# mfalxa/fakepta

Hardware: AMD Instinct MI355X
Metric: residual samples/sec (TOA×realization) for 100-psr HD GWB; % FP64 peak (higher is better)
Workload: dtype f64

## Files before the change

### fakepta_amd/csrc/fused_sched.h

```cpp
#pragma once
#include <cstdint>

#if defined(__HIPCC__)
#define FPTA_SCHED_HD __host__ __device__
#else
#define FPTA_SCHED_HD
#endif

namespace fpta {

constexpr int kFusedShapeAny = 0;
constexpr int kFusedShapeGenLoad = 1;
constexpr int kFusedShapeLoad = 2;
constexpr int kFusedSlotAny = -1, kFusedSlotNone = 0, kFusedSlotGen = 1, kFusedSlotLoad = 2;
FPTA_SCHED_HD constexpr int fused_shape_nsig(int shape) {
  return shape == kFusedShapeGenLoad ? 2 : shape == kFusedShapeLoad ? 1 : 0;
}
FPTA_SCHED_HD constexpr int fused_shape_slot(int shape, int s, int i) {
  return shape == kFusedShapeAny       ? kFusedSlotAny
         : shape == kFusedShapeGenLoad ? (i == 0 ? kFusedSlotGen : (s == 0 && i == 1 ? kFusedSlotLoad : kFusedSlotNone))
                                       : (s == 0 && i == 0 ? kFusedSlotLoad : kFusedSlotNone);
}

FPTA_SCHED_HD constexpr int fused_shape_match(int n_sig, const int32_t* n_terms, const int32_t (*kind)[2]) {
  return n_sig == 2 && n_terms[0] == 2 && kind[0][0] == 0 && kind[0][1] == 1 && n_terms[1] == 1 && kind[1][0] == 0
             ? kFusedShapeGenLoad
         : n_sig == 1 && n_terms[0] == 1 && kind[0][0] == 1 ? kFusedShapeLoad
                                                            : kFusedShapeAny;
}

FPTA_SCHED_HD constexpr int32_t fused_ksteps(int32_t nm, int par) { return (((nm + (par ? 0 : 1)) >> 1) + 3) >> 2; }
FPTA_SCHED_HD constexpr int32_t fused_groups(int32_t nm) { return (fused_ksteps(nm, 0) + 1) >> 1; }

FPTA_SCHED_HD constexpr int32_t fused_iterations(int32_t ng0, int32_t ng1) { return ng0 > ng1 ? ng0 : ng1; }
FPTA_SCHED_HD constexpr bool fused_steps(int32_t jng, int32_t g) { return g < jng; }
FPTA_SCHED_HD constexpr bool fused_draw_loads(int32_t ng_s, int32_t g, bool last) { return last || g + 1 < ng_s; }
FPTA_SCHED_HD constexpr bool fused_draws(int32_t ng_s, int32_t g, bool last, bool nx) { return last ? nx : g + 1 < ng_s; }
FPTA_SCHED_HD constexpr int32_t fused_draw_group(int32_t g, bool last) { return last ? 0 : g + 1; }

}

#undef FPTA_SCHED_HD
```

### fakepta_amd/csrc/grid_fused.hip

```cpp
#include <hip/hip_runtime.h>
#include <hip/hip_ext.h>
#include <algorithm>
#include <atomic>
#include <type_traits>

#include "fused_device.h"

namespace fpta {

#ifndef FPTA_FUSED_DFT_PRIO
#define FPTA_FUSED_DFT_PRIO 3
#endif
#ifndef FPTA_HALF_STORE16
#define FPTA_HALF_STORE16 0
#endif
#ifndef FPTA_HALF_AHEAD
#define FPTA_HALF_AHEAD 2
#endif
constexpr int kFusedHalfAhead = FPTA_HALF_AHEAD;
#ifndef FPTA_HALF_PIN
#define FPTA_HALF_PIN 0
#endif

#ifndef FPTA_FUSED_CUT
#define FPTA_FUSED_CUT 0
#endif

namespace {

template <int NS>
struct FusedOps {
  int c;
  i32x4 ci;
  dbl2 b[NS];
  int row[NS];
};
template <int NS>
struct FusedOpsH {
  int c;
  i32x4 ci;
  dbl2 b[2][NS / 2];
  int row[2][NS];
};

__device__ __forceinline__ uint32_t dpp_u32_xor1(uint32_t x) {
  return (uint32_t)__builtin_amdgcn_update_dpp(0, (int)x, 0xB1, 0xF, 0xF, false);
}
__device__ __forceinline__ void bm_half(uint32_t wl, uint32_t wa, double& zc, double& zs) {
  double sn, cs;
  const double r = bm_sqrt(-2.0 * bm_log_u32(wl));
  bm_sincos2pi_u32(wa, sn, cs);
  zc = r * cs;
  zs = r * sn;
}
__device__ __forceinline__ void fused_mix_tile(const FusedMix& m, int k, int rg, int pg, int lane) {
  constexpr int NT = kFusedMixGroup / 16;
  const int lr = lane & 15, lg = lane >> 4;
  const int r = 16 * rg + lr;
  const bool rv = r < m.n_real;
  const uint64_t g = (uint64_t)(m.real0 + r);
  const int p0 = kFusedMixGroup * pg;
  int qe[NT];
  int qmax = 0;
#pragma unroll
  for (int t = 0; t < NT; ++t) {
    const int pt = p0 + 16 * t;
    qe[t] = pt < m.P ? min(m.lower ? min(m.P, pt + 16) : m.P, m.n_q) : 0;
    qmax = max(qmax, qe[t]);
  }
  d4 acc[NT][2];
#pragma unroll
  for (int t = 0; t < NT; ++t) acc[t][0] = acc[t][1] = d4{0.0, 0.0, 0.0, 0.0};
  const double* __restrict__ lt = m.LT + p0 + lr;
  const bool paired = (m.real0 & 1) == 0;
  const int e = lr & 1;
  const uint32_t ctr3 = (uint32_t)(g >> 1);
  for (int q0 = 0; q0 < qmax; q0 += 8) {
    double a0[NT], a1[NT];
#pragma unroll
    for (int t = 0; t < NT; ++t) {
      a0[t] = q0 < qe[t] ? ld_global(lt + (int64_t)(q0 + lg) * m.lt_ld + 16 * t) : 0.0;
      a1[t] = q0 + 4 < qe[t] ? ld_global(lt + (int64_t)(q0 + 4 + lg) * m.lt_ld + 16 * t) : 0.0;
    }
    double zc0, zs0, zc1, zs1;
    if (paired) {
      const u32x4 v = philox4x32_10({(uint32_t)k, (uint32_t)(q0 + 4 * e + lg), (uint32_t)m.seg, ctr3}, m.k0, m.k1);
      const uint32_t r0 = dpp_u32_xor1(e ? v.x : v.z), r1 = dpp_u32_xor1(e ? v.y : v.w);
      bm_half(e ? r0 : v.x, e ? r1 : v.y, zc0, zs0);
      bm_half(e ? v.z : r0, e ? v.w : r1, zc1, zs1);
    } else {
      gp_normal2((uint32_t)k, (uint32_t)(q0 + lg), (uint32_t)m.seg, g, m.k0, m.k1, zc0, zs0);
      gp_normal2((uint32_t)k, (uint32_t)(q0 + 4 + lg), (uint32_t)m.seg, g, m.k0, m.k1, zc1, zs1);
    }
    const bool ok0 = rv && q0 + lg < m.n_q, ok1 = rv && q0 + 4 + lg < m.n_q;
    zc0 = ok0 ? zc0 : 0.0;
    zs0 = ok0 ? zs0 : 0.0;
    zc1 = ok1 ? zc1 : 0.0;
    zs1 = ok1 ? zs1 : 0.0;
#pragma unroll
    for (int t = 0; t < NT; ++t)
      if (q0 < qe[t]) {
        acc[t][0] = __builtin_amdgcn_mfma_f64_16x16x4f64(a0[t], zc0, acc[t][0], 0, 0, 0);
        acc[t][1] = __builtin_amdgcn_mfma_f64_16x16x4f64(a0[t], zs0, acc[t][1], 0, 0, 0);
      }
#pragma unroll
    for (int t = 0; t < NT; ++t)
      if (q0 + 4 < qe[t]) {
        acc[t][0] = __builtin_amdgcn_mfma_f64_16x16x4f64(a1[t], zc1, acc[t][0], 0, 0, 0);
        acc[t][1] = __builtin_amdgcn_mfma_f64_16x16x4f64(a1[t], zs1, acc[t][1], 0, 0, 0);
      }
  }
  const double am = ld_global(m.amp + k);
#pragma unroll
  for (int t = 0; t < NT; ++t)
#pragma unroll
    for (int h = 0; h < 2; ++h)
#pragma unroll
      for (int gg = 0; gg < 4; ++gg) {
        const int p = p0 + 16 * t + lg + 4 * gg;
        if (p < m.P) m.coef[((int64_t)p * m.K + m.col0 + 2 * k + h) * m.R_pad + r] = am * acc[t][h][gg];
      }
}

}

template <int NQ, bool ODD, bool GEN, bool HALF, int SHAPE>
__device__ __forceinline__ void grid_fused_body(const SynthArgs& a, const GridBand& band, const FusedArgs& f,
                                                int32_t n_rb, int32_t n_items) {
  static_assert(kFusedTerms == 2 && kFusedMaxSig == 2, "fused_shape_slot's slots and signals (c0, c1)");
  static_assert(SHAPE == kFusedShapeAny || GEN == (SHAPE == kFusedShapeGenLoad), "a shape fixes whether terms are drawn");
  static_assert(kFusedReal == 32 && kFusedPitch == 32 && kFusedGroupModes * kFusedReal / 2 == 64 * kFusedDW,
                "two realization tiles; one (mode, realization pair) of a 16-mode group per DFT lane");
  static_assert(!HALF || (NQ % 4 == 0 && kGridTT == 2 * kFusedHalfTT), "half bands: whole row groups, two halves");
  extern __shared__ __attribute__((aligned(16))) double lds[];
  const FusedQueue queue(n_items, f.queue);
  const int wave = __builtin_amdgcn_readfirstlane(threadIdx.x >> 6);
  const int lane = threadIdx.x & 63;
  const int lr = lane & 15, lg = lane >> 4;
  double* __restrict__ ring = lds + f.ring_off;
  uint32_t* sync = (uint32_t*)(ring + 2 * kFusedMaxSig * kFusedSlot);
  volatile int* qitem = (volatile int*)(sync + 4);
  if (threadIdx.x == 0) {
    *sync = 0u;
    ((volatile int*)sync)[8] = 0;
    ((volatile int*)sync)[9] = 0;
    qitem[0] = queue.fetch();
    qitem[1] = qitem[0] >= 0 ? queue.fetch() : -1;
  }
  __syncthreads();
  auto item_of = [&](int k) { return __builtin_amdgcn_readfirstlane(qitem[k & 3]); };
  auto finish = [&]() {
    if (threadIdx.x == 0) {
      __threadfence();
      const uint32_t done = __hip_atomic_fetch_add(f.queue + 8, 1u, __ATOMIC_ACQ_REL, __HIP_MEMORY_SCOPE_AGENT);
      if (done == gridDim.x - 1)
        for (int i = 0; i < kFusedQueueWords; ++i)
          __hip_atomic_store(f.queue + i, 0u, __ATOMIC_RELAXED, __HIP_MEMORY_SCOPE_AGENT);
    }
  };
  auto mix_tiles = [&]() {
    if (f.mix.n_tiles <= 0) return;
    __builtin_amdgcn_s_setprio(0);
    const int n_pg = (f.mix.P + kFusedMixGroup - 1) / kFusedMixGroup, n_rg = f.mix.R_pad >> 4;
    for (;;) {
      int t = 0;
      if (lane == 0)
        t = (int)__hip_atomic_fetch_add(f.queue + kFusedMixWord, 1u, __ATOMIC_RELAXED, __HIP_MEMORY_SCOPE_AGENT);
      t = __builtin_amdgcn_readfirstlane(t);
      if (t >= f.mix.n_tiles) break;
      const int pg = t % n_pg, kr = t / n_pg;
      const int k = kr / n_rg;
      fused_mix_tile(f.mix, k, kr - k * n_rg, pg, lane);
    }
  };
  if (item_of(0) < 0) {
    finish();
    return;
  }

  volatile int* ccnt = (volatile int*)(sync + 8);
  struct Geo {
    int p, r0, c0, n;
    int64_t toa0;
    bool valid;
  };
  auto geo = [&](int k) {
    Geo g;
    const int item = item_of(k);
    g.valid = item >= 0;
    const int it = g.valid ? item : 0;
    g.p = it / n_rb;
    g.r0 = (it - g.p * n_rb) * kFusedReal;
    g.c0 = ld_uniform(f.psr_c0 + g.p);
    g.n = g.valid ? ld_uniform(f.psr_c0 + g.p + 1) - g.c0 : 0;
    g.toa0 = ld_uniform(a.offs + g.p);
    return g;
  };
  auto ticket = [&](int k) {
    int t = 0;
    if (lane == 0)
      t = __hip_atomic_fetch_add((int*)ccnt + (k & 1), 1, __ATOMIC_RELAXED, __HIP_MEMORY_SCOPE_WORKGROUP);
    return __builtin_amdgcn_readfirstlane(t);
  };
  auto lane_now = [&]() {
    int v = lane;
    asm volatile("" : "+v"(v));
    return v;
  };
  using Ops = typename std::conditional<HALF, FusedOpsH<NQ>, FusedOps<NQ>>::type;
  using OpsJ = typename std::conditional<HALF, FusedOpsH<NQ>, FusedOps<(NQ < 8 ? NQ : 8)>>::type;
  auto load_half = [&](int cc, auto& o, int ln) {
    {
      constexpr int NS = sizeof(o.row[0]) / sizeof(o.row[0][0]);
      o.c = cc;
      o.ci = *(const i32x4*)(f.h.chunks + cc);
      const int lgo = ln >> 4, lro = ln & 15;
#pragma unroll
      for (int h = 0; h < 2; ++h) {
        const i32x4* __restrict__ rt = (const i32x4*)(f.h.lrows + (((int64_t)cc * 2 + h) * 4 + lgo) * f.h.fq);
#pragma unroll
        for (int q4 = 0; q4 < NS / 4; ++q4) {
          const i32x4 r4 = rt[q4];
          o.row[h][4 * q4] = r4.x;
          o.row[h][4 * q4 + 1] = r4.y;
          o.row[h][4 * q4 + 2] = r4.z;
          o.row[h][4 * q4 + 3] = r4.w;
        }
        const double* __restrict__ wp =
            f.h.wd + ((int64_t)cc * 2 + h) * f.h.vmax * kFusedHalfTT + (lgo * kFusedHalfTT + lro) * 2;
#pragma unroll
        for (int qp = 0; qp < NS / 2; ++qp) o.b[h][qp] = *(const dbl2*)(wp + qp * 8 * kFusedHalfTT);
      }
    }
  };
  auto load_full = [&](int cc, auto& o, int ln) {
    constexpr int NS = sizeof(o.row) / sizeof(o.row[0]);
    o.c = cc;
    o.ci = *(const i32x4*)(band.chunks + cc);
    const int lgo = ln >> 4, lro = ln & 15;
    const i32x4* __restrict__ rt = (const i32x4*)(f.lrows + ((int64_t)cc * 4 + lgo) * f.fq);
    const double* __restrict__ wp = band.wd + ((int64_t)cc * band.vmax + lgo) * kGridTT + 2 * lro;
#pragma unroll
    for (int q4 = 0; q4 < NS / 4; ++q4) {
      const i32x4 r4 = rt[q4];
      o.row[4 * q4] = r4.x;
      o.row[4 * q4 + 1] = r4.y;
      o.row[4 * q4 + 2] = r4.z;
      o.row[4 * q4 + 3] = r4.w;
    }
#pragma unroll
    for (int q = 0; q < NS; ++q) o.b[q] = *(const dbl2*)(wp + 4 * kGridTT * q);
  };
  auto load = [&](int cc, auto& o, int ln) {
    if constexpr (HALF)
      load_half(cc, o, ln);
    else
      load_full(cc, o, ln);
  };
  auto process_half = [&](const Geo& g, const auto& cur, auto& pf, int ln) {
    constexpr int NS = sizeof(cur.row[0]) / sizeof(cur.row[0][0]);
    const int lg = ln >> 4, lr = ln & 15;
    const int lds_lane = 2 * lr;
    const int ty = __builtin_amdgcn_readfirstlane(cur.ci.y), tc = __builtin_amdgcn_readfirstlane(cur.ci.z);
    const int nqw = __builtin_amdgcn_readfirstlane(cur.ci.w);
    const int nq[2] = {nqw & 0xFFFF, nqw >> 16};
    FPTA_DCHECK(nq[0] > 0, "k_grid_fused half band steps", nq[0], 1 << 20);
    d4 acc[2][2];
#pragma unroll
    for (int h = 0; h < 2; ++h)
#pragma unroll
      for (int i = 0; i < 2; ++i) acc[h][i] = d4{0.0, 0.0, 0.0, 0.0};
    {
      constexpr int DA = kFusedHalfAhead;
      const int nqm = min(max(nq[0], nq[1]), NS);
      dbl2 an[2][NS];
      auto rd = [&](int q) {
#pragma unroll
        for (int h = 0; h < 2; ++h) an[h][q] = *(const dbl2*)(lds + cur.row[h][q] * kFusedPitch + lds_lane);
      };
#pragma unroll
      for (int q = 0; q < DA && q < NS; ++q) rd(q);
#pragma unroll
      for (int q = 0; q < NS; ++q) {
        if (q < nqm) {
          if (q + DA < NS) rd(q + DA);
          if (FPTA_HALF_PIN) __builtin_amdgcn_sched_barrier(0);
          const double b0 = (q & 1) ? cur.b[0][q >> 1].y : cur.b[0][q >> 1].x;
          const double b1 = (q & 1) ? cur.b[1][q >> 1].y : cur.b[1][q >> 1].x;
          acc[0][0] = __builtin_amdgcn_mfma_f64_16x16x4f64(an[0][q].x, b0, acc[0][0], 0, 0, 0);
          acc[0][1] = __builtin_amdgcn_mfma_f64_16x16x4f64(an[0][q].y, b0, acc[0][1], 0, 0, 0);
          acc[1][0] = __builtin_amdgcn_mfma_f64_16x16x4f64(an[1][q].x, b1, acc[1][0], 0, 0, 0);
          acc[1][1] = __builtin_amdgcn_mfma_f64_16x16x4f64(an[1][q].y, b1, acc[1][1], 0, 0, 0);
        }
      }
    }
    pf.lap(1);
#pragma unroll
    for (int h = 0; h < 2; ++h)
      for (int q = NS; q < nq[h]; ++q) {
        const int64_t hc = (int64_t)cur.c * 2 + h;
        const int row = f.h.lrows[(hc * 4 + lg) * f.h.fq + q];
        const double bv = f.h.wd[hc * f.h.vmax * kFusedHalfTT + fused_half_weight_index(4 * q + lg, lr)];
        const dbl2 av = *(const dbl2*)(lds + row * kFusedPitch + lds_lane);
        acc[h][0] = __builtin_amdgcn_mfma_f64_16x16x4f64(av.x, bv, acc[h][0], 0, 0, 0);
        acc[h][1] = __builtin_amdgcn_mfma_f64_16x16x4f64(av.y, bv, acc[h][1], 0, 0, 0);
      }
    pf.lap(4);
    __builtin_amdgcn_sched_barrier(0);
    const int64_t t0 = g.toa0 + ty;
    if ((FPTA_FUSED_CUT & 8) && acc[0][0][0] != -1.25e300) return;
    if (FPTA_HALF_STORE16 && tc == kGridTT && g.r0 + kFusedReal <= a.n_real && ((t0 | a.ldo) & 1) == 0 &&
        a.ldo < ((int64_t)1 << 26)) {
      const bool odd = lr & 1;
      const uint32_t vo = (uint32_t)(((int64_t)2 * lg * a.ldo + (odd ? 15 + lr : lr)) * 8);
      const char* base = (const char*)(a.out + t0 + (int64_t)g.r0 * a.ldo);
#pragma unroll
      for (int i = 0; i < 2; ++i)
#pragma unroll
        for (int gg = 0; gg < 4; ++gg) {
          const double send = odd ? acc[0][i][gg] : acc[1][i][gg];
          const double recv = dpp_xor1(send);
          const dbl2 v = odd ? dbl2{recv, acc[1][i][gg]} : dbl2{acc[0][i][gg], recv};
          __builtin_nontemporal_store(v, (dbl2*)((char*)base + (int64_t)(8 * gg + i) * a.ldo * 8 + vo));
        }
    } else if (tc == kGridTT && g.r0 + kFusedReal <= a.n_real && a.ldo < ((int64_t)1 << 26)) {
      const uint32_t vo = (uint32_t)(((int64_t)2 * lg * a.ldo + lr) * 8);
      const char* base = (const char*)(a.out + t0 + (int64_t)g.r0 * a.ldo);
#pragma unroll
      for (int h = 0; h < 2; ++h)
#pragma unroll
        for (int i = 0; i < 2; ++i)
#pragma unroll
          for (int gg = 0; gg < 4; ++gg)
            __builtin_nontemporal_store(acc[h][i][gg],
                                        (double*)((char*)base + ((int64_t)(8 * gg + i) * a.ldo + 16 * h) * 8 + vo));
    } else {
#pragma unroll
      for (int h = 0; h < 2; ++h) {
        if (16 * h + lr >= tc) continue;
#pragma unroll
        for (int i = 0; i < 2; ++i)
#pragma unroll
          for (int gg = 0; gg < 4; ++gg) {
            const int r = g.r0 + 2 * (lg + 4 * gg) + i;
            if (r < a.n_real) a.out[t0 + 16 * h + lr + (int64_t)r * a.ldo] = acc[h][i][gg];
          }
      }
    }
    pf.lap(2);
  };
  auto process_full = [&](const Geo& g, const auto& cur, auto& pf, int ln) {
    constexpr int NS = sizeof(cur.row) / sizeof(cur.row[0]);
    const int lg = ln >> 4, lr = ln & 15;
    const int lds_lane = 2 * lr;
    const int ty = __builtin_amdgcn_readfirstlane(cur.ci.y), tc = __builtin_amdgcn_readfirstlane(cur.ci.z);
    const int nq = __builtin_amdgcn_readfirstlane(cur.ci.w) >> 2;
    FPTA_DCHECK(nq > 0, "k_grid_fused band steps", nq, 1 << 20);
    d4 acc[2][2];
#pragma unroll
    for (int e = 0; e < 2; ++e)
#pragma unroll
      for (int i = 0; i < 2; ++i) acc[e][i] = d4{0.0, 0.0, 0.0, 0.0};
    {
      dbl2 an = *(const dbl2*)(lds + cur.row[0] * kFusedPitch + lds_lane);
#pragma unroll
      for (int q = 0; q < NS; ++q) {
        if (q < nq) {
          const dbl2 av = an;
          if (q + 1 < NS) an = *(const dbl2*)(lds + cur.row[q + 1] * kFusedPitch + lds_lane);
          const dbl2 bv = cur.b[q];
          acc[0][0] = __builtin_amdgcn_mfma_f64_16x16x4f64(av.x, bv.x, acc[0][0], 0, 0, 0);
          acc[0][1] = __builtin_amdgcn_mfma_f64_16x16x4f64(av.y, bv.x, acc[0][1], 0, 0, 0);
          acc[1][0] = __builtin_amdgcn_mfma_f64_16x16x4f64(av.x, bv.y, acc[1][0], 0, 0, 0);
          acc[1][1] = __builtin_amdgcn_mfma_f64_16x16x4f64(av.y, bv.y, acc[1][1], 0, 0, 0);
        }
      }
    }
    pf.lap(1);
    for (int q = NS; q < nq; ++q) {
      const int v = 4 * q + lg;
      const int row = f.lrows[((int64_t)cur.c * 4 + lg) * f.fq + q];
      const dbl2 bv = *(const dbl2*)(band.wd + ((int64_t)cur.c * band.vmax + v) * kGridTT + 2 * lr);
      const dbl2 av = *(const dbl2*)(lds + row * kFusedPitch + lds_lane);
      acc[0][0] = __builtin_amdgcn_mfma_f64_16x16x4f64(av.x, bv.x, acc[0][0], 0, 0, 0);
      acc[0][1] = __builtin_amdgcn_mfma_f64_16x16x4f64(av.y, bv.x, acc[0][1], 0, 0, 0);
      acc[1][0] = __builtin_amdgcn_mfma_f64_16x16x4f64(av.x, bv.y, acc[1][0], 0, 0, 0);
      acc[1][1] = __builtin_amdgcn_mfma_f64_16x16x4f64(av.y, bv.y, acc[1][1], 0, 0, 0);
    }
    pf.lap(4);
    __builtin_amdgcn_sched_barrier(0);
    const int64_t t0 = g.toa0 + ty;
    if ((FPTA_FUSED_CUT & 8) && acc[0][0][0] != -1.25e300) return;
    if (FPTA_HALF_STORE16 && tc == kGridTT && g.r0 + kFusedReal <= a.n_real && ((t0 | a.ldo) & 1) == 0 &&
        a.ldo < ((int64_t)1 << 26)) {
      const uint32_t vo = (uint32_t)(((int64_t)2 * lg * a.ldo + 2 * lr) * 8);
      const char* base = (const char*)(a.out + t0 + (int64_t)g.r0 * a.ldo);
#pragma unroll
      for (int i = 0; i < 2; ++i)
#pragma unroll
        for (int gg = 0; gg < 4; ++gg)
          __builtin_nontemporal_store(dbl2{acc[0][i][gg], acc[1][i][gg]},
                                      (dbl2*)((char*)base + (int64_t)(8 * gg + i) * a.ldo * 8 + vo));
    } else {
      InterpTile<2> t;
      t.c = cur.c;
      t.p = g.p;
      t.r0 = g.r0;
      t.y = ty;
      t.cnt = tc;
      t.nq = nq;
      interp_store_rows<2>(a, a.out, t, acc);
    }
    pf.lap(2);
  };
  auto process = [&](const Geo& g, const auto& cur, auto& pf, int ln) {
    if constexpr (HALF)
      process_half(g, cur, pf, ln);
    else
      process_full(g, cur, pf, ln);
  };

  if (wave >= kFusedIW) {
    const int dw = wave - kFusedIW;
    __builtin_amdgcn_s_setprio(FPTA_FUSED_DFT_PRIO);
    constexpr int kNSig = fused_shape_nsig(SHAPE);
    const int n_sig = kNSig ? kNSig : f.n_sig;
    int js = -1, jrc = 0;
    {
      int j = dw;
#pragma unroll
      for (int s = 0; s < kFusedMaxSig; ++s) {
        if (s < n_sig && js < 0 && j < f.s[s].n_rc) {
          js = s;
          jrc = j;
        }
        if (s < n_sig) j -= f.s[s].n_rc;
      }
    }
    js = __builtin_amdgcn_readfirstlane(js);
    jrc = __builtin_amdgcn_readfirstlane(jrc);
    Prof pf;
    pf.start();
    uint32_t epoch = 0;
    auto dsync = [&]() {
      fused_wait_lgkm0();
      if (lane == 0) __hip_atomic_fetch_add(sync, 1u, __ATOMIC_RELAXED, __HIP_MEMORY_SCOPE_WORKGROUP);
      epoch += kFusedDW;
      while ((uint32_t)__builtin_amdgcn_readfirstlane(
                 (int)__hip_atomic_load(sync, __ATOMIC_RELAXED, __HIP_MEMORY_SCOPE_WORKGROUP)) < epoch)
        __builtin_amdgcn_s_sleep(1);
    };
    int ng[kFusedMaxSig];
#pragma unroll
    for (int s = 0; s < kFusedMaxSig; ++s) ng[s] = s < n_sig ? fused_groups(f.s[s].nm) : 0;
    const int n_it = fused_iterations(ng[0], ng[1]);
    const FusedSig& jf = f.s[js < 0 ? 0 : js];
    const int64_t jts = (int64_t)jf.ntq * jf.ldq, jld4 = 4 * (int64_t)jf.ldq;
    auto jtq_now = [&]() {
      const int ln = lane_now();
      return jf.tq + (int64_t)(ln >> 4) * jf.ldq + 32 * jrc + 2 * (ln & 15);
    };
    const int jnq0 = fused_ksteps(jf.nm, 0), jnq1 = fused_ksteps(jf.nm, 1);
    const int jng = js < 0 ? 0 : fused_groups(jf.nm);
    d4 C[2][2][2], S[2][2][2];
    struct DrawIn {
      dbl2 x0[kFusedTerms], x1[kFusedTerms];
    };
    std::integral_constant<int, 0> c0;
    std::integral_constant<int, 1> c1;
    auto draw_load = [&](auto sc, int g, int p, int r0, DrawIn& in) {
      constexpr int s = decltype(sc)::value;
      const FusedSig& fs = f.s[s];
      const int didx = dw * 64 + lane_now(), dmm = didx >> 4, drl = 2 * (didx & 15);
      const int m = kFusedGroupModes * g + dmm, r = r0 + drl;
      auto slot = [&](auto ic) {
        constexpr int i = decltype(ic)::value, kind = fused_shape_slot(SHAPE, s, i);
        if constexpr (kind == kFusedSlotGen) {
          const int nmi = fs.term_nm[i], mi = min(m, nmi - 1);
          in.x0[i] = ld_global((const dbl2*)(fs.term_amp[i] + (int64_t)p * nmi + (mi & ~1)));
        } else if constexpr (kind == kFusedSlotLoad) {
          const int mi = min(m, fs.term_nm[i] - 1);
          const double* src0 = a.coef + ((int64_t)p * a.K + fs.term_col0[i] + 2 * mi) * a.R_pad + r;
          in.x0[i] = ld_global((const dbl2*)src0);
          in.x1[i] = ld_global((const dbl2*)(src0 + a.R_pad));
        } else if constexpr (kind == kFusedSlotAny) {
          const bool on = i < fs.n_terms;
          const int nmi = on ? fs.term_nm[i] : 2;
          const int mi = min(m, nmi - 1);
          const double* src0;
          int64_t step;
          if (on && fs.term_kind[i] == 1) {
            src0 = a.coef + ((int64_t)p * a.K + fs.term_col0[i] + 2 * mi) * a.R_pad + r;
            step = a.R_pad;
          } else {
            src0 = (on ? fs.term_amp[i] : a.coef) + (int64_t)p * nmi + (mi & ~1);
            step = 0;
          }
          in.x0[i] = ld_global((const dbl2*)src0);
          in.x1[i] = ld_global((const dbl2*)(src0 + step));
        }
      };
      slot(c0);
      slot(c1);
    };
    auto draw_finish = [&](auto sc, int g, int p, int r0, double* __restrict__ slot_s, const DrawIn& in) {
      constexpr int s = decltype(sc)::value;
      const FusedSig& fs = f.s[s];
      const int didx = dw * 64 + lane_now(), dmm = didx >> 4, drl = 2 * (didx & 15);
      const int m = kFusedGroupModes * g + dmm, r = r0 + drl;
      const uint64_t gr = (uint64_t)(f.real0 + r);
      double bc[2] = {0.0, 0.0}, bs[2] = {0.0, 0.0};
      bool first = true;
      auto add = [&](bool use, const double (&pc)[2], const double (&ps)[2]) {
#pragma unroll
        for (int h = 0; h < 2; ++h) {
          bc[h] = use ? (first ? pc[h] : bc[h] + pc[h]) : bc[h];
          bs[h] = use ? (first ? ps[h] : bs[h] + ps[h]) : bs[h];
        }
        first = first && !use;
      };
      const bool ok0 = r < a.n_real, ok1 = r + 1 < a.n_real;
      auto normals = [&](int seg, double (&z)[4]) {
        uint32_t k0 = f.k0, k1 = f.k1;
        if (SHAPE != kFusedShapeAny) asm volatile("" : "+s"(k0), "+s"(k1));
        if (!ODD) {
          gp_pair2((uint32_t)m, (uint32_t)p, (uint32_t)seg, gr, k0, k1, z);
        } else {
          gp_normal2((uint32_t)m, (uint32_t)p, (uint32_t)seg, gr, k0, k1, z[0], z[1]);
          gp_normal2((uint32_t)m, (uint32_t)p, (uint32_t)seg, gr + 1, k0, k1, z[2], z[3]);
        }
        z[0] = ok0 ? z[0] : 0.0;
        z[1] = ok0 ? z[1] : 0.0;
        z[2] = ok1 ? z[2] : 0.0;
        z[3] = ok1 ? z[3] : 0.0;
      };
      auto term = [&](auto ic) {
        constexpr int i = decltype(ic)::value, kind = fused_shape_slot(SHAPE, s, i);
        if (kind == kFusedSlotNone || (kind == kFusedSlotAny && i >= fs.n_terms)) return;
        double pc[2], ps[2];
        if (kind == kFusedSlotGen || (kind == kFusedSlotAny && GEN && fs.term_kind[i] == 0)) {
          double z[4];
          normals(fs.term_seg[i], z);
          const double amp = (m & 1) ? in.x0[i].y : in.x0[i].x;
          pc[0] = opaque(amp * z[0]);
          ps[0] = opaque(amp * z[1]);
          pc[1] = opaque(amp * z[2]);
          ps[1] = opaque(amp * z[3]);
        } else {
          pc[0] = in.x0[i].x;
          pc[1] = in.x0[i].y;
          ps[0] = in.x1[i].x;
          ps[1] = in.x1[i].y;
        }
        add(m < fs.nm && m < fs.term_nm[i], pc, ps);
      };
      term(c0);
      term(c1);
      for (int i = kFusedTerms; SHAPE == kFusedShapeAny && i < fs.n_terms; ++i) {
        const int mi = min(m, fs.term_nm[i] - 1);
        double pc[2], ps[2];
        if (GEN && fs.term_kind[i] == 0) {
          double z[4];
          normals(fs.term_seg[i], z);
          const double amp = ld_global(fs.term_amp[i] + (int64_t)p * fs.term_nm[i] + mi);
          pc[0] = opaque(amp * z[0]);
          ps[0] = opaque(amp * z[1]);
          pc[1] = opaque(amp * z[2]);
          ps[1] = opaque(amp * z[3]);
        } else {
          const double* cp = a.coef + ((int64_t)p * a.K + fs.term_col0[i] + 2 * mi) * a.R_pad + r;
          const dbl2 vc = ld_global((const dbl2*)cp), vs = ld_global((const dbl2*)(cp + a.R_pad));
          pc[0] = vc.x;
          pc[1] = vc.y;
          ps[0] = vs.x;
          ps[1] = vs.y;
        }
        add(m < fs.nm && m < fs.term_nm[i], pc, ps);
      }
      double* __restrict__ dst = slot_s + 2 * (dmm * kFusedReal + drl);
      *(dbl2*)dst = dbl2{bc[0], bs[0]};
      *(dbl2*)(dst + 2) = dbl2{bc[1], bs[1]};
    };
    auto slot_of = [&](int k, int s) { return ring + ((k & 1) * kFusedMaxSig + s) * kFusedSlot; };
    struct Tabs {
      dbl2 ac[2][2], as[2][2];
    };
    auto tables = [&](int g, Tabs& tb) {
#pragma unroll
      for (int h2 = 0; h2 < 2; ++h2) {
        const int q = max(0, min(2 * g + h2, jnq0 - 1));
#pragma unroll
        for (int par = 0; par < 2; ++par) {
          const double* __restrict__ tc = jtq_now() + (int64_t)(2 * par) * jts + q * jld4;
          tb.ac[h2][par] = ld_global((const dbl2*)tc);
          tb.as[h2][par] = ld_global((const dbl2*)(tc + jts));
        }
      }
    };
    auto steps = [&](int slot, int g, const Tabs& tb) {
      const double* __restrict__ bsrc = slot_of(slot, js);
#pragma unroll
      for (int h2 = 0; h2 < 2; ++h2) {
        const int q = 2 * g + h2;
#pragma unroll
        for (int par = 0; par < 2; ++par) {
          if (q >= (par ? jnq1 : jnq0)) continue;
          const dbl2 ac = tb.ac[h2][par], as = tb.as[h2][par];
          const double* bm = bsrc + 2 * ((2 * (4 * h2 + lg) + par) * kFusedReal + lr);
          const dbl2 b[2] = {*(const dbl2*)bm, *(const dbl2*)(bm + 2 * 16)};
#pragma unroll
          for (int t = 0; t < 2; ++t) {
            C[par][0][t] = __builtin_amdgcn_mfma_f64_16x16x4f64(ac.x, b[t].x, C[par][0][t], 0, 0, 0);
            C[par][1][t] = __builtin_amdgcn_mfma_f64_16x16x4f64(ac.y, b[t].x, C[par][1][t], 0, 0, 0);
            S[par][0][t] = __builtin_amdgcn_mfma_f64_16x16x4f64(as.x, b[t].y, S[par][0][t], 0, 0, 0);
            S[par][1][t] = __builtin_amdgcn_mfma_f64_16x16x4f64(as.y, b[t].y, S[par][1][t], 0, 0, 0);
          }
        }
      }
    };
    int sb = 0;
    auto build = [&](int k) {
      const int item = item_of(k);
      const int p = item / n_rb, r0 = (item - p * n_rb) * kFusedReal;
      const int item1n = item_of(k + 1);
      const bool nx = item1n >= 0;
      const int item1 = nx ? item1n : item;
      const int p1 = item1 / n_rb, r1 = (item1 - p1 * n_rb) * kFusedReal;
#pragma unroll
      for (int par = 0; par < 2; ++par)
#pragma unroll
        for (int h = 0; h < 2; ++h)
#pragma unroll
          for (int t = 0; t < 2; ++t) C[par][h][t] = S[par][h][t] = d4{0.0, 0.0, 0.0, 0.0};
      if (k == 0) {
        auto first = [&](auto sc) {
          constexpr int s = decltype(sc)::value;
          if (s >= n_sig) return;
          DrawIn in;
          draw_load(sc, 0, p, r0, in);
          draw_finish(sc, 0, p, r0, slot_of(sb, s), in);
        };
        first(c0);
        first(c1);
        pf.lap(6);
        dsync();
        pf.lap(2);
      }
      constexpr bool kAny = SHAPE == kFusedShapeAny;
      for (int g = 0; g < n_it; ++g) {
        const bool last = g + 1 == n_it;
        const int dp = last ? p1 : p, dr = last ? r1 : r0;
        Tabs tb;
        if (kAny) tables(g, tb);
        DrawIn in[kFusedMaxSig];
        auto load = [&](auto sc) {
          constexpr int s = decltype(sc)::value;
          if (kAny || (s < kNSig && fused_draw_loads(ng[s], g, last)))
            draw_load(sc, last ? 0 : min(g + 1, max(ng[s], 1) - 1), dp, dr, in[s]);
        };
        load(c0);
        load(c1);
        if (!kAny && fused_steps(jng, g)) tables(g, tb);
        pf.lap(0);
        if (fused_steps(jng, g)) steps(sb + g, g, tb);
        pf.lap(1);
        auto finish_draw = [&](auto sc) {
          constexpr int s = decltype(sc)::value;
          if (s < n_sig && fused_draws(ng[s], g, last, nx))
            draw_finish(sc, fused_draw_group(g, last), dp, dr, slot_of(sb + g + 1, s), in[s]);
        };
        finish_draw(c0);
        finish_draw(c1);
        pf.lap(6);
        if (!kAny) fused_wait_vm0();
        dsync();
        pf.lap(2);
        pf.count(5);
      }
      sb = (sb + n_it) & 1;
    };
    auto write_grid = [&]() {
      if (js >= 0) {
        const int j0 = 32 * jrc;
        const int nf = jf.nf, Q = nf >> 2, H = nf >> 1;
        double* __restrict__ gcol = lds + (int64_t)jf.lrow0 * kFusedPitch + lr;
#pragma unroll
        for (int h = 0; h < 2; ++h)
#pragma unroll
          for (int gg = 0; gg < 4; ++gg) {
            const int j = j0 + 2 * (lg + 4 * gg) + h;
            if (j > Q) continue;
#pragma unroll
            for (int t = 0; t < 2; ++t) {
              const double oc = C[0][h][t][gg], os = S[0][h][t][gg], ec = C[1][h][t][gg], es = S[1][h][t][gg];
              const double pe = ec + es, me = ec - es, po = oc + os, mo = oc - os;
              gcol[j * kFusedPitch + 16 * t] = pe + po;
              gcol[(H + j) * kFusedPitch + 16 * t] = pe - po;
              if (j > 0 && j < Q) {
                gcol[(H - j) * kFusedPitch + 16 * t] = me - mo;
                gcol[(nf - j) * kFusedPitch + 16 * t] = me + mo;
              }
            }
          }
      }
      fused_wait_lgkm0();
    };
    auto join = [&](int k) {
      if (FPTA_FUSED_CUT & 6) return;
      const Geo g = geo(k);
      auto take = [&]() {
        if (__builtin_amdgcn_readfirstlane(ccnt[k & 1]) >= g.n - f.join_reserve) return -1;
        const int t = ticket(k);
        return t < g.n ? t : -1;
      };
      int t = take();
      if (t < 0) return;
      OpsJ o0, o1;
      load(g.c0 + t, o0, lane_now());
      for (;;) {
        t = take();
        load(t >= 0 ? g.c0 + t : o0.c, o1, lane_now());
        process(g, o0, pf, lane_now());
        pf.count(7);
        if (t < 0) return;
        t = take();
        load(t >= 0 ? g.c0 + t : o1.c, o0, lane_now());
        process(g, o1, pf, lane_now());
        pf.count(7);
        if (t < 0) return;
      }
    };
    auto barrier_a = [&](int k) {
      fused_barrier();
      pf.lap(4);
      if (dw == 0 && lane == 0) ccnt[k & 1] = 0;
    };
    for (int k = -1;; ++k) {
      const bool next = item_of(k + 1) >= 0;
      if (dw == 0 && lane == 0) qitem[(k + 3) & 3] = item_of(k + 2) >= 0 ? queue.fetch() : -1;
      if (k >= 0) join(k);
      if (!next) break;
      if (!(FPTA_FUSED_CUT & 1)) build(k + 1);
      if (k >= 0) barrier_a(k);
      write_grid();
      pf.lap(3);
      fused_barrier();
      pf.lap(4);
    }
    pf.flush(f.prof, wave);
  } else {
  Prof pf;
  pf.start();
  fused_barrier();
  pf.lap(3);
  int k = 0;
  Geo g0 = geo(0), g1 = geo(1);
  bool ex0 = false, ex1 = false;
  auto next = [&](int& kn) {
    if (!ex0) {
      const int t = ticket(k);
      if (t < g0.n) {
        kn = k;
        return g0.c0 + t;
      }
      ex0 = true;
    }
    if (!ex1 && g1.valid) {
      const int t = ticket(k + 1);
      if (t < g1.n) {
        kn = k + 1;
        return g1.c0 + t;
      }
      ex1 = true;
    }
    kn = -1;
    return -1;
  };
  auto step = [&](Ops& cur, Ops& nxt, int& kc) {
    pf.lap(6);
    int kn;
    const int cn = next(kn);
    load(cn >= 0 ? cn : cur.c, nxt, lane);
    pf.lap(0);
    pf.count(5);
    if (!(FPTA_FUSED_CUT & 2)) process(g0, cur, pf, lane);
    kc = kn;
  };
  Ops o0, o1;
  int kc;
  {
    const int cc = next(kc);
    load(cc >= 0 ? cc : g0.c0, o0, lane);
  }
  for (;;) {
    while (kc == k) {
      step(o0, o1, kc);
      if (kc != k) {
        o0 = o1;
        break;
      }
      step(o1, o0, kc);
    }
    if (!g1.valid) break;
    fused_wait_lgkm0();
    pf.lap(6);
    fused_barrier();
    fused_barrier();
    pf.lap(3);
    ++k;
    g0 = g1;
    g1 = geo(k + 1);
    ex0 = ex1;
    ex1 = false;
    if (kc < 0) {
      const int cc = next(kc);
      load(cc >= 0 ? cc : g0.c0, o0, lane);
    }
  }
  pf.flush(f.prof, wave);
  }
  mix_tiles();
  fused_barrier();
  if (wave < kFusedIW) finish();
}

template <int NQ, bool ODD, bool GEN, bool HALF>
__global__ __launch_bounds__(64 * (kFusedIW + kFusedDW), 1) void k_grid_fused(SynthArgs a, GridBand band, FusedArgs f,
                                                                             int32_t n_rb, int32_t n_items) {
  grid_fused_body<NQ, ODD, GEN, HALF, GEN ? kFusedShapeGenLoad : kFusedShapeLoad>(a, band, f, n_rb, n_items);
}
template <int NQ, bool ODD, bool GEN, bool HALF>
__global__ __launch_bounds__(64 * (kFusedIW + kFusedDW), 1) void k_grid_fused_any(SynthArgs a, GridBand band,
                                                                                 FusedArgs f, int32_t n_rb,
                                                                                 int32_t n_items) {
  grid_fused_body<NQ, ODD, GEN, HALF, kFusedShapeAny>(a, band, f, n_rb, n_items);
}

#ifndef FPTA_FUSED_SHAPES
#define FPTA_FUSED_SHAPES 1
#endif
static int fused_shape_of(const FusedArgs& f) {
  int32_t n_terms[kFusedMaxSig], kind[kFusedMaxSig][2];
  for (int s = 0; s < kFusedMaxSig; ++s) {
    n_terms[s] = f.s[s].n_terms;
    kind[s][0] = f.s[s].term_kind[0];
    kind[s][1] = f.s[s].term_kind[1];
  }
  return FPTA_FUSED_SHAPES ? fused_shape_match(f.n_sig, n_terms, kind) : kFusedShapeAny;
}

hipError_t launch_grid_fused(hipStream_t st, const SynthArgs& a, const GridBand& band, const FusedArgs& f,
                             int32_t nq_max, size_t lds_bytes, hipEvent_t ev0, hipEvent_t ev1, bool half,
                             int* kernel_out, int* shape_out) {
  if (band.n_chunks <= 0 || band.vmax < 4 || f.join_reserve < 0 || band.vmax % 4 != 0 || a.R_pad % kFusedReal != 0 || a.w_on ||
      a.accumulate || a.part || !f.lrows || !f.psr_c0 || f.n_sig <= 0 || f.n_sig > kFusedMaxSig ||
      lds_bytes > (size_t)kFusedLdsMax || nq_max <= 0 || f.ring_off < 0 || f.fq < kFusedNQ || f.fq % 4 != 0 ||
      !f.queue || (size_t)(f.ring_off + 2 * kFusedMaxSig * kFusedSlot) * sizeof(double) + 48 > lds_bytes)
    return hipErrorInvalidValue;
  if (half && (!f.h.chunks || !f.h.lrows || !f.h.wd || f.h.fq < kFusedHalfNQ || f.h.fq % 4 != 0 || f.h.vmax < 8 ||
               f.h.vmax % 8 != 0))
    return hipErrorInvalidValue;
  int jobs = 0;
  for (int s = 0; s < f.n_sig; ++s) {
    const FusedSig& fs = f.s[s];
    const int nq = fused_ksteps(fs.nm, 0);
    if (fs.nf % 4 != 0 || !fs.tq || fs.n_rc != (fs.nf / 4 + 32) / 32 || fs.ldq < 32 * fs.n_rc || 4 * nq > fs.ntq ||
        fs.n_terms <= 0 || fs.n_terms > kDftGenTerms || fs.lrow0 < 0 || (fs.lrow0 + fs.nf) * kFusedPitch > f.ring_off)
      return hipErrorInvalidValue;
    for (int i = 0; i < fs.n_terms; ++i)
      if (fs.term_nm[i] <= 0 || fs.term_nm[i] > fs.nm || (fs.term_kind[i] == 0 && (!fs.term_amp[i] || fs.term_nm[i] % 2)) ||
          (fs.term_kind[i] == 1 && (!a.coef || fs.term_col0[i] < 0 || fs.term_col0[i] + 2 * fs.term_nm[i] > a.K)))
        return hipErrorInvalidValue;
    jobs += fs.n_rc;
  }
  if (jobs > kFusedDW) return hipErrorInvalidValue;
  const FusedMix& m = f.mix;
  if (m.n_tiles != 0 &&
      (m.n_tiles < 0 || !m.LT || !m.amp || !m.coef || m.P <= 0 || m.P > kFusedMixMaxP || m.lt_ld < 16 * ((m.P + 15) / 16) ||
       m.lt_rows < 4 * ((m.P + 3) / 4) || m.n_q <= 0 || m.n_q > m.P || m.nm <= 0 || m.R_pad <= 0 ||
       m.R_pad % 16 != 0 || m.n_real <= 0 || m.n_real > m.R_pad || (int64_t)m.n_tiles != (int64_t)m.nm * (m.R_pad / 16) * ((m.P + kFusedMixGroup - 1) / kFusedMixGroup) ||
       m.col0 < 0 || m.col0 + 2 * m.nm > m.K || m.real0 < 0 || m.real0 + m.n_real > ((int64_t)1 << 32)))
    return hipErrorInvalidValue;
  const int32_t n_rb = a.R_pad / kFusedReal;
  const int64_t items = (int64_t)a.P * n_rb;
  if (items > 0x7FFFFFFF || items <= 0) return hipErrorInvalidValue;
  int dev = 0;
  if (hipGetDevice(&dev) != hipSuccess || dev < 0 || dev >= 64) return hipErrorInvalidDevice;
  static std::atomic<int> n_cus[64];
  static std::atomic<bool> attr_set[64][2][kFusedKernels];
  int n_cu = n_cus[dev].load(std::memory_order_relaxed);
  if (n_cu <= 0) {
    if (hipDeviceGetAttribute(&n_cu, hipDeviceAttributeMultiprocessorCount, dev) != hipSuccess || n_cu <= 0) n_cu = 256;
    n_cus[dev].store(n_cu, std::memory_order_relaxed);
  }
  const int64_t cus = f.cu_pct > 0 && f.cu_pct < 100 ? std::max<int64_t>(8, (int64_t)n_cu * f.cu_pct / 100) : n_cu;
  const int64_t grid = std::min<int64_t>((items + 7) / 8 * 8, (cus + 7) / 8 * 8);
  bool gen = false;
  for (int s = 0; s < f.n_sig; ++s)
    for (int i = 0; i < f.s[s].n_terms; ++i) gen = gen || f.s[s].term_kind[i] == 0;
  const bool odd = gen && (f.real0 & 1);
  const int ki = half ? 6 + (gen ? 1 + odd : 0) : (nq_max <= 8 ? 0 : 3) + (gen ? 1 + odd : 0);
  using K = void (*)(SynthArgs, GridBand, FusedArgs, int32_t, int32_t);
  static const K kernels[2][kFusedKernels] = {
      {k_grid_fused_any<8, false, false, false>, k_grid_fused_any<8, false, true, false>,
       k_grid_fused_any<8, true, true, false>, k_grid_fused_any<12, false, false, false>,
       k_grid_fused_any<12, false, true, false>, k_grid_fused_any<12, true, true, false>,
       k_grid_fused_any<kFusedHalfNQ, false, false, true>, k_grid_fused_any<kFusedHalfNQ, false, true, true>,
       k_grid_fused_any<kFusedHalfNQ, true, true, true>},
      {k_grid_fused<8, false, false, false>, k_grid_fused<8, false, true, false>, k_grid_fused<8, true, true, false>,
       k_grid_fused<12, false, false, false>, k_grid_fused<12, false, true, false>, k_grid_fused<12, true, true, false>,
       k_grid_fused<kFusedHalfNQ, false, false, true>, k_grid_fused<kFusedHalfNQ, false, true, true>,
       k_grid_fused<kFusedHalfNQ, true, true, true>}};
  const int shaped = fused_shape_of(f) == (gen ? kFusedShapeGenLoad : kFusedShapeLoad) ? 1 : 0;
  const K kernel = kernels[shaped][ki];
  if (!attr_set[dev][shaped][ki].load(std::memory_order_acquire)) {
    hipError_t e = hipFuncSetAttribute((const void*)kernel, hipFuncAttributeMaxDynamicSharedMemorySize, kFusedLdsMax);
    if (e != hipSuccess) return e;
    attr_set[dev][shaped][ki].store(true, std::memory_order_release);
  }
  FusedArgs fa = f;
  for (int s = f.n_sig; s < kFusedMaxSig; ++s) fa.s[s] = f.s[0];
  (void)hipGetLastError();
  int32_t n_rb_arg = n_rb, items_arg = (int32_t)items;
  void* args[] = {(void*)&a, (void*)&band, (void*)&fa, (void*)&n_rb_arg, (void*)&items_arg};
  const hipError_t e = hipExtLaunchKernel((const void*)kernel, dim3((unsigned)grid),
                                          dim3(64 * (kFusedIW + kFusedDW)), args, lds_bytes, st, ev0, ev1, 0);
  if (e == hipSuccess && kernel_out) *kernel_out = ki;
  if (e == hipSuccess && shape_out) *shape_out = shaped ? (gen ? kFusedShapeGenLoad : kFusedShapeLoad) : kFusedShapeAny;
  return e;
}

}
```

### fakepta_amd/csrc/philox.h

```cpp
#pragma once
#include <hip/hip_runtime.h>
#include <stdint.h>

namespace fpta {

struct u32x4 {
  uint32_t x, y, z, w;
};

__host__ __device__ __forceinline__ u32x4 philox4x32_10(u32x4 c, uint32_t k0, uint32_t k1) {
#pragma unroll
  for (int i = 0; i < 10; ++i) {
    const uint64_t p0 = (uint64_t)0xD2511F53u * c.x;
    const uint64_t p1 = (uint64_t)0xCD9E8D57u * c.z;
    u32x4 n;
#if defined(__HIP_DEVICE_COMPILE__) && __has_builtin(__builtin_amdgcn_bitop3_b32)
    n.x = __builtin_amdgcn_bitop3_b32((uint32_t)(p1 >> 32), c.y, k0, 0x96);
    n.z = __builtin_amdgcn_bitop3_b32((uint32_t)(p0 >> 32), c.w, k1, 0x96);
#else
    n.x = (uint32_t)(p1 >> 32) ^ c.y ^ k0;
    n.z = (uint32_t)(p0 >> 32) ^ c.w ^ k1;
#endif
    n.y = (uint32_t)p1;
    n.w = (uint32_t)p0;
    c = n;
    k0 += 0x9E3779B9u;
    k1 += 0xBB67AE85u;
  }
  return c;
}

__device__ __forceinline__ void box_muller(u32x4 v, double& z0, double& z1) {
  const uint64_t a = (uint64_t)v.x | ((uint64_t)v.y << 32);
  const uint64_t b = (uint64_t)v.z | ((uint64_t)v.w << 32);
  const double u1 = (double)((a >> 11) + 1ull) * 0x1.0p-53;
  const double u2 = (double)(b >> 11) * 0x1.0p-53;
  const double r = sqrt(-2.0 * log(u1));
  double s, c;
  sincospi(2.0 * u2, &s, &c);
  z0 = r * c;
  z1 = r * s;
}

__device__ __forceinline__ double bm_log_u32(uint32_t a) {
  const double n = (double)a + 1.0;
  int e;
  double m = frexp(n, &e);
  if (m < 0.7071067811865476) {
    m *= 2.0;
    e -= 1;
  }
  const double k = (double)(e - 32);
  const double num = m - 1.0, den = m + 1.0;
  double rc = __builtin_amdgcn_rcp(den);
  rc = fma(rc, fma(-den, rc, 1.0), rc);
  rc = fma(rc, fma(-den, rc, 1.0), rc);
  double s = num * rc;
  s = fma(fma(-den, s, num), rc, s);
  const double s2 = s * s;
  const double p =
      s2 * (1.0 / 3.0 +
            s2 * (1.0 / 5.0 + s2 * (1.0 / 7.0 + s2 * (1.0 / 9.0 + s2 * (1.0 / 11.0 + s2 * (1.0 / 13.0 + s2 * (1.0 / 15.0)))))));
  const double lm = 2.0 * s + 2.0 * s * p;
  return k * 6.93147180369123816490e-01 + (k * 1.90821492927058770002e-10 + lm);
}

__device__ __forceinline__ void bm_sincos2pi_u32(uint32_t b, double& sn, double& cs) {
  const double u = (double)b * 0x1.0p-32;
  const double q = rint(4.0 * u);
  const double y = u - 0.25 * q;
  const double a = y * 6.283185307179586;
  const double x2 = a * a;
  const double sa =
      a + a * x2 *
              (-1.0 / 6.0 +
               x2 * (1.0 / 120.0 +
                     x2 * (-1.0 / 5040.0 + x2 * (1.0 / 362880.0 + x2 * (-1.0 / 39916800.0 + x2 * (1.0 / 6227020800.0))))));
  const double ca =
      1.0 + x2 * (-1.0 / 2.0 +
                  x2 * (1.0 / 24.0 +
                        x2 * (-1.0 / 720.0 +
                              x2 * (1.0 / 40320.0 +
                                    x2 * (-1.0 / 3628800.0 + x2 * (1.0 / 479001600.0 + x2 * (-1.0 / 87178291200.0)))))));
  const int qi = (int)q & 3;
  const bool sw = (qi & 1) != 0;
  const double s0 = sw ? ca : sa;
  const double c0 = sw ? sa : ca;
  sn = __longlong_as_double(__double_as_longlong(s0) ^ ((long long)(qi & 2) << 62));
  cs = __longlong_as_double(__double_as_longlong(c0) ^ ((long long)((qi + 1) & 2) << 62));
}

__device__ __forceinline__ double bm_sqrt(double x) {
  const double y = __builtin_amdgcn_rsq(x);
  double g = x * y, h = 0.5 * y;
  const double r = fma(-g, h, 0.5);
  g = fma(g, r, g);
  h = fma(h, r, h);
  g = fma(fma(-g, g, x), h, g);
  return x > 0.0 ? g : 0.0;
}

__device__ __forceinline__ void normals4(u32x4 v, double (&z)[4]) {
  double s, c;
  const double r0 = bm_sqrt(-2.0 * bm_log_u32(v.x));
  bm_sincos2pi_u32(v.y, s, c);
  z[0] = r0 * c;
  z[1] = r0 * s;
#ifndef FPTA_NORMALS4_SPLIT
#define FPTA_NORMALS4_SPLIT 1
#endif
  if (FPTA_NORMALS4_SPLIT) __builtin_amdgcn_sched_barrier(0);
  const double r1 = bm_sqrt(-2.0 * bm_log_u32(v.z));
  bm_sincos2pi_u32(v.w, s, c);
  z[2] = r1 * c;
  z[3] = r1 * s;
}

__device__ __forceinline__ void gp_normal2(uint32_t k, uint32_t p, uint32_t seg, uint64_t g, uint32_t k0, uint32_t k1,
                                           double& zc, double& zs) {
  const u32x4 v = philox4x32_10({k, p, seg, (uint32_t)(g >> 1)}, k0, k1);
  const bool odd = (g & 1) != 0;
  double s, c;
  const double r = bm_sqrt(-2.0 * bm_log_u32(odd ? v.z : v.x));
  bm_sincos2pi_u32(odd ? v.w : v.y, s, c);
  zc = r * c;
  zs = r * s;
}
__device__ __forceinline__ void gp_pair2(uint32_t k, uint32_t p, uint32_t seg, uint64_t g_even, uint32_t k0,
                                         uint32_t k1, double (&z)[4]) {
  normals4(philox4x32_10({k, p, seg, (uint32_t)(g_even >> 1)}, k0, k1), z);
}

constexpr uint32_t kWhitePsrWord = 0xFFFFFFFFu;
constexpr uint32_t kWhiteStream = 0xFFFFFFF0u;
constexpr uint32_t kEcorrStream = 0xFFFFFFF1u;
constexpr uint32_t kDenseStream = 0xFFFFFFF2u;

}

namespace fpta {
__device__ __forceinline__ double quad_normal(uint64_t i, uint32_t stream, uint64_t g, uint32_t k0, uint32_t k1) {
  double z[4];
  normals4(philox4x32_10({(uint32_t)(i >> 1), kWhitePsrWord, stream, (uint32_t)(g >> 1)}, k0, k1), z);
  const double lo = (g & 1) ? z[1] : z[0], hi = (g & 1) ? z[3] : z[2];
  return (i & 1) ? hi : lo;
}
__device__ __forceinline__ void quad4(uint64_t i_even, uint32_t stream, uint64_t g_even, uint32_t k0, uint32_t k1,
                                      double (&z)[4]) {
  normals4(philox4x32_10({(uint32_t)(i_even >> 1), kWhitePsrWord, stream, (uint32_t)(g_even >> 1)}, k0, k1), z);
}
}
```

Baseline: 382.1 billion.

## Interleave Box-Muller pairs in lockstep and skip normal draws for padded waves

Adds a lockstep variant of the four-normal Box-Muller transform that interleaves the two log/sincos/sqrt chains stage by stage. This exposes instruction-level parallelism across the otherwise serial FP64 dependency chains and is used in the specialised fused shapes. It also skips Philox and normal generation for waves whose mode index lies entirely past the term's mode count, zero-filling instead. The cost is higher register pressure from the interleaving, plus a divergent branch in the generator path.

```diff
diff --git a/fakepta_amd/csrc/fused_sched.h b/fakepta_amd/csrc/fused_sched.h
--- a/fakepta_amd/csrc/fused_sched.h
+++ b/fakepta_amd/csrc/fused_sched.h
@@ -38,6 +38,11 @@
 FPTA_SCHED_HD constexpr bool fused_draws(int32_t ng_s, int32_t g, bool last, bool nx) { return last ? nx : g + 1 < ng_s; }
 FPTA_SCHED_HD constexpr int32_t fused_draw_group(int32_t g, bool last) { return last ? 0 : g + 1; }
 
+FPTA_SCHED_HD constexpr bool fused_wave_padded(int32_t group, int32_t dw, int32_t nm) { return 16 * group + 4 * dw >= nm; }
+FPTA_SCHED_HD constexpr bool fused_wave_draws(int32_t ng_s, int32_t g, bool last, bool nx, int32_t dw, int32_t nm) {
+  return fused_draws(ng_s, g, last, nx) && !fused_wave_padded(fused_draw_group(g, last), dw, nm);
+}
+
 }
 
 #undef FPTA_SCHED_HD
diff --git a/fakepta_amd/csrc/grid_fused.hip b/fakepta_amd/csrc/grid_fused.hip
--- a/fakepta_amd/csrc/grid_fused.hip
+++ b/fakepta_amd/csrc/grid_fused.hip
@@ -20,6 +20,13 @@
 constexpr int kFusedHalfAhead = FPTA_HALF_AHEAD;
 #ifndef FPTA_HALF_PIN
 #define FPTA_HALF_PIN 0
+#endif
+
+#ifndef FPTA_FUSED_LOCKSTEP
+#define FPTA_FUSED_LOCKSTEP 1
+#endif
+#ifndef FPTA_FUSED_SKIP_PAD
+#define FPTA_FUSED_SKIP_PAD 1
 #endif
 
 #ifndef FPTA_FUSED_CUT
@@ -524,7 +531,12 @@
         uint32_t k0 = f.k0, k1 = f.k1;
         if (SHAPE != kFusedShapeAny) asm volatile("" : "+s"(k0), "+s"(k1));
         if (!ODD) {
-          gp_pair2((uint32_t)m, (uint32_t)p, (uint32_t)seg, gr, k0, k1, z);
+          if (SHAPE != kFusedShapeAny && FPTA_FUSED_LOCKSTEP) {
+            normals4_lockstep(
+                philox4x32_10({(uint32_t)m, (uint32_t)p, (uint32_t)seg, (uint32_t)(gr >> 1)}, k0, k1), z);
+          } else {
+            gp_pair2((uint32_t)m, (uint32_t)p, (uint32_t)seg, gr, k0, k1, z);
+          }
         } else {
           gp_normal2((uint32_t)m, (uint32_t)p, (uint32_t)seg, gr, k0, k1, z[0], z[1]);
           gp_normal2((uint32_t)m, (uint32_t)p, (uint32_t)seg, gr + 1, k0, k1, z[2], z[3]);
@@ -539,8 +551,9 @@
         if (kind == kFusedSlotNone || (kind == kFusedSlotAny && i >= fs.n_terms)) return;
         double pc[2], ps[2];
         if (kind == kFusedSlotGen || (kind == kFusedSlotAny && GEN && fs.term_kind[i] == 0)) {
-          double z[4];
-          normals(fs.term_seg[i], z);
+          double z[4] = {0.0, 0.0, 0.0, 0.0};
+          if (!(FPTA_FUSED_SKIP_PAD && kind == kFusedSlotGen && fused_wave_padded(g, dw, fs.term_nm[i])))
+            normals(fs.term_seg[i], z);
           const double amp = (m & 1) ? in.x0[i].y : in.x0[i].x;
           pc[0] = opaque(amp * z[0]);
           ps[0] = opaque(amp * z[1]);
diff --git a/fakepta_amd/csrc/philox.h b/fakepta_amd/csrc/philox.h
--- a/fakepta_amd/csrc/philox.h
+++ b/fakepta_amd/csrc/philox.h
@@ -8,24 +8,29 @@
   uint32_t x, y, z, w;
 };
 
+constexpr uint32_t kPhiloxW0 = 0x9E3779B9u, kPhiloxW1 = 0xBB67AE85u;
+__host__ __device__ __forceinline__ u32x4 philox4x32_round(u32x4 c, uint32_t k0, uint32_t k1) {
+  const uint64_t p0 = (uint64_t)0xD2511F53u * c.x;
+  const uint64_t p1 = (uint64_t)0xCD9E8D57u * c.z;
+  u32x4 n;
+#if defined(__HIP_DEVICE_COMPILE__) && __has_builtin(__builtin_amdgcn_bitop3_b32)
+  n.x = __builtin_amdgcn_bitop3_b32((uint32_t)(p1 >> 32), c.y, k0, 0x96);
+  n.z = __builtin_amdgcn_bitop3_b32((uint32_t)(p0 >> 32), c.w, k1, 0x96);
+#else
+  n.x = (uint32_t)(p1 >> 32) ^ c.y ^ k0;
+  n.z = (uint32_t)(p0 >> 32) ^ c.w ^ k1;
+#endif
+  n.y = (uint32_t)p1;
+  n.w = (uint32_t)p0;
+  return n;
+}
+
 __host__ __device__ __forceinline__ u32x4 philox4x32_10(u32x4 c, uint32_t k0, uint32_t k1) {
 #pragma unroll
   for (int i = 0; i < 10; ++i) {
-    const uint64_t p0 = (uint64_t)0xD2511F53u * c.x;
-    const uint64_t p1 = (uint64_t)0xCD9E8D57u * c.z;
-    u32x4 n;
-#if defined(__HIP_DEVICE_COMPILE__) && __has_builtin(__builtin_amdgcn_bitop3_b32)
-    n.x = __builtin_amdgcn_bitop3_b32((uint32_t)(p1 >> 32), c.y, k0, 0x96);
-    n.z = __builtin_amdgcn_bitop3_b32((uint32_t)(p0 >> 32), c.w, k1, 0x96);
-#else
-    n.x = (uint32_t)(p1 >> 32) ^ c.y ^ k0;
-    n.z = (uint32_t)(p0 >> 32) ^ c.w ^ k1;
-#endif
-    n.y = (uint32_t)p1;
-    n.w = (uint32_t)p0;
-    c = n;
-    k0 += 0x9E3779B9u;
-    k1 += 0xBB67AE85u;
+    c = philox4x32_round(c, k0, k1);
+    k0 += kPhiloxW0;
+    k1 += kPhiloxW1;
   }
   return c;
 }
@@ -116,6 +121,124 @@
   z[3] = r1 * s;
 }
 
+__device__ __forceinline__ void normals4_lockstep(u32x4 v, double (&z)[4]) {
+  const uint32_t wa[2] = {v.x, v.z}, wb[2] = {v.y, v.w};
+  double m[2], k[2], num[2], den[2], rc[2], s[2], s2[2], p[2], u[2], q[2], a[2], x2[2], ps[2], pc[2], sa[2], ca[2];
+  int e[2];
+#pragma unroll
+  for (int j = 0; j < 2; ++j) {
+    const double n = (double)wa[j] + 1.0;
+    m[j] = frexp(n, &e[j]);
+    u[j] = (double)wb[j] * 0x1.0p-32;
+  }
+#pragma unroll
+  for (int j = 0; j < 2; ++j) {
+    if (m[j] < 0.7071067811865476) {
+      m[j] *= 2.0;
+      e[j] -= 1;
+    }
+    q[j] = rint(4.0 * u[j]);
+  }
+#pragma unroll
+  for (int j = 0; j < 2; ++j) {
+    k[j] = (double)(e[j] - 32);
+    num[j] = m[j] - 1.0;
+    den[j] = m[j] + 1.0;
+    const double y = u[j] - 0.25 * q[j];
+    a[j] = y * 6.283185307179586;
+  }
+#pragma unroll
+  for (int j = 0; j < 2; ++j) {
+    rc[j] = __builtin_amdgcn_rcp(den[j]);
+    x2[j] = a[j] * a[j];
+  }
+#pragma unroll
+  for (int j = 0; j < 2; ++j) {
+    rc[j] = fma(rc[j], fma(-den[j], rc[j], 1.0), rc[j]);
+    ps[j] = -1.0 / 39916800.0 + x2[j] * (1.0 / 6227020800.0);
+    pc[j] = 1.0 / 479001600.0 + x2[j] * (-1.0 / 87178291200.0);
+  }
+#pragma unroll
+  for (int j = 0; j < 2; ++j) {
+    rc[j] = fma(rc[j], fma(-den[j], rc[j], 1.0), rc[j]);
+    ps[j] = 1.0 / 362880.0 + x2[j] * ps[j];
+    pc[j] = -1.0 / 3628800.0 + x2[j] * pc[j];
+  }
+#pragma unroll
+  for (int j = 0; j < 2; ++j) {
+    s[j] = num[j] * rc[j];
+    ps[j] = -1.0 / 5040.0 + x2[j] * ps[j];
+    pc[j] = 1.0 / 40320.0 + x2[j] * pc[j];
+  }
+#pragma unroll
+  for (int j = 0; j < 2; ++j) {
+    s[j] = fma(fma(-den[j], s[j], num[j]), rc[j], s[j]);
+    ps[j] = 1.0 / 120.0 + x2[j] * ps[j];
+    pc[j] = -1.0 / 720.0 + x2[j] * pc[j];
+  }
+#pragma unroll
+  for (int j = 0; j < 2; ++j) {
+    s2[j] = s[j] * s[j];
+    ps[j] = -1.0 / 6.0 + x2[j] * ps[j];
+    pc[j] = 1.0 / 24.0 + x2[j] * pc[j];
+  }
+#pragma unroll
+  for (int j = 0; j < 2; ++j) {
+    p[j] = 1.0 / 13.0 + s2[j] * (1.0 / 15.0);
+    sa[j] = a[j] + a[j] * x2[j] * ps[j];
+    pc[j] = -1.0 / 2.0 + x2[j] * pc[j];
+  }
+#pragma unroll
+  for (int j = 0; j < 2; ++j) {
+    p[j] = 1.0 / 11.0 + s2[j] * p[j];
+    ca[j] = 1.0 + x2[j] * pc[j];
+  }
+  double sn[2], cs[2];
+#pragma unroll
+  for (int j = 0; j < 2; ++j) {
+    p[j] = 1.0 / 9.0 + s2[j] * p[j];
+    const int qi = (int)q[j] & 3;
+    const bool sw = (qi & 1) != 0;
+    const double s0 = sw ? ca[j] : sa[j];
+    const double c0 = sw ? sa[j] : ca[j];
+    sn[j] = __longlong_as_double(__double_as_longlong(s0) ^ ((long long)(qi & 2) << 62));
+    cs[j] = __longlong_as_double(__double_as_longlong(c0) ^ ((long long)((qi + 1) & 2) << 62));
+  }
+#pragma unroll
+  for (int j = 0; j < 2; ++j) p[j] = 1.0 / 7.0 + s2[j] * p[j];
+#pragma unroll
+  for (int j = 0; j < 2; ++j) p[j] = 1.0 / 5.0 + s2[j] * p[j];
+#pragma unroll
+  for (int j = 0; j < 2; ++j) p[j] = s2[j] * (1.0 / 3.0 + s2[j] * p[j]);
+  double x[2], y[2], g[2], h[2], r[2];
+#pragma unroll
+  for (int j = 0; j < 2; ++j) {
+    const double lm = 2.0 * s[j] + 2.0 * s[j] * p[j];
+    x[j] = -2.0 * (k[j] * 6.93147180369123816490e-01 + (k[j] * 1.90821492927058770002e-10 + lm));
+  }
+#pragma unroll
+  for (int j = 0; j < 2; ++j) y[j] = __builtin_amdgcn_rsq(x[j]);
+#pragma unroll
+  for (int j = 0; j < 2; ++j) {
+    g[j] = x[j] * y[j];
+    h[j] = 0.5 * y[j];
+  }
+#pragma unroll
+  for (int j = 0; j < 2; ++j) r[j] = fma(-g[j], h[j], 0.5);
+#pragma unroll
+  for (int j = 0; j < 2; ++j) {
+    g[j] = fma(g[j], r[j], g[j]);
+    h[j] = fma(h[j], r[j], h[j]);
+  }
+#pragma unroll
+  for (int j = 0; j < 2; ++j) {
+    g[j] = fma(fma(-g[j], g[j], x[j]), h[j], g[j]);
+    const double rr = x[j] > 0.0 ? g[j] : 0.0;
+    z[2 * j] = rr * cs[j];
+    z[2 * j + 1] = rr * sn[j];
+  }
+}
+
 __device__ __forceinline__ void gp_normal2(uint32_t k, uint32_t p, uint32_t seg, uint64_t g, uint32_t k0, uint32_t k1,
                                            double& zc, double& zs) {
   const u32x4 v = philox4x32_10({k, p, seg, (uint32_t)(g >> 1)}, k0, k1);
```

Result: faster. 386.9 billion (median of 5 runs) (+1.2%).
